# tub-rip/dvs_mcemvs

Hardware: AMD Instinct MI355X
Metric: Mevents/s into DSI (346x260x100) + DSI-fuse GB/s (higher is better)
Workload: dtype f32; 1 GPU; stereo (2-cam) synthetic DSEC-like rig, 10000000 events/cam per GPU, 346x260x100 DSI, harmonic camera fusion + arg-max; vote_algo=2, bands=10, band_rows=26, chunks=1, block_threads=1024, lds_bytes=74736, packed_lanes=7, parallelism=1 GPU, collective=none (1 rank), launched_by=single process, n_points=5000

## Files before the change

### dvs_mcemvs_amd/csrc/dsi_engine.cpp

```cpp
#include "../../include/dsi_engine.h"

#include <hip/hip_runtime.h>
#include <rccl/rccl.h>

#include <dlfcn.h>

#include <algorithm>
#include <atomic>
#include <chrono>
#include <cmath>
#include <cstdarg>
#include <cstdio>
#include <cstdlib>
#include <cstring>
#include <map>
#include <mutex>
#include <new>
#include <string>
#include <utility>
#include <vector>

#include "dsi_host.hpp"
#include "dsi_kernels.h"

// ... 295 lines not shown
    int algo = DSI_VOTE_AUTO;
    int want_band_rows = 0, want_chunks = 0, want_block = 0;
    int want_packed = -1;
    bool keep_z0 = false;
    dsi_vote_info_t info{};
    DevBuf<float> centers, H, Rt_tmp, conf, depth;
    DevBuf<unsigned long long> partials;
    DevBuf<float2> xy;
    DevBuf<dsi::EvRec> sxy;
    DevBuf<unsigned long long> seam;
    DevBuf<uint32_t> nvalid, cuts, gcuts;
    size_t cuts_inline_min_packets = 8192;
    bool info_cuts_inline = false;
    DevBuf<uint8_t> spk;
    DevBuf<uint16_t> rowstart;
    DevBuf<dsi::PlaneCoef> coef;
    DevBuf<uint8_t> idx, conf8, mask, idx_filtered;
    DevBuf<uint32_t> minmax;
    bool depth_valid = false;
    bool filtered_valid = false;
    PcBuffers pc;
    struct BatchTables {
        DevBuf<float> centers;
        DevBuf<dsi::EvRec> sxy;
        DevBuf<uint32_t> nvalid, cuts;
        DevBuf<uint16_t> rowstart;
        DevBuf<dsi::PlaneCoef> coef;
        void release()
        {
            centers.release();
// ... 331 lines not shown
    dsi_grid* g = m->grid;
    const dsi::Geom& geom = m->geom;
    dsi::BandPlan bp{};
    int algo = m->algo;
    const bool can_band = plan_bands(m, np, &bp);
    if (algo == DSI_VOTE_AUTO) algo = can_band ? DSI_VOTE_LDS_BANDS : DSI_VOTE_GLOBAL_ATOMIC;
    if (algo == DSI_VOTE_LDS_BANDS && !can_band)
        return fail(DSI_ERR_INVALID, "grid rows of %d floats do not fit the LDS band kernel", geom.nx);

    m->info = dsi_vote_info_t{};
    m->info.algo = algo;
    m->info.n_packets = np;
    m->depth_valid = false;

    if (algo == DSI_VOTE_GLOBAL_ATOMIC) {
        if (int rc = stage_a()) return rc;
        if (int rc = prep_end(m, ps)) return rc;
        if (!accumulate) HIP_TRY(hipMemsetAsync(g->data, 0, g->n * sizeof(float), ctx->stream));
        VoteTimer vt(m);
        HIP_TRY(dsi::launch_vote_global(ctx->stream, xy, centers, (int)np, m->planes_dev, geom, g->data));
        vt.stop();
        return vote_done(m);
    }

    if ((np + 1) * dsi::kPacket * sizeof(dsi::EvRec) > 0xffffffffull) {
        if (bp.packed == 1 || bp.packed == 7) bp.packed = 3;
        if (bp.packed == 8) return fail(DSI_ERR_INVALID, "lane mapping 8 (paired cells) addresses records with 32 bits: %zu packets are too many", np);
        if (bp.packed == 4) bp.packed = 2;
        if (bp.packed == 5) bp.packed = 6;
    }

    m->info.bands = bp.bands;
    m->info.band_rows = bp.band_rows;
    m->info.chunks = bp.chunks;
    m->info.block_threads = bp.block_threads;
    m->info.lds_bytes = bp.lds_bytes;
    m->info.packed = bp.packed;
    m->info.group_packets = bp.group_packets;
    if (np == 0) {
        if (int rc = prep_end(m, ps)) return rc;
        if (!accumulate) HIP_TRY(hipMemsetAsync(g->data, 0, g->n * sizeof(float), ctx->stream));
        return vote_done(m);
    }
    HIP_TRY(m->sxy.reserve(np * dsi::kPacket + 1));
    HIP_TRY(m->nvalid.reserve(np + (size_t)geom.nz + 9));
    HIP_TRY(m->rowstart.reserve(np * (size_t)(geom.ny + 2 * bp.row_pad + 3) + 2));
    HIP_TRY(m->coef.reserve(np * geom.nz + 1));
    bp.rs_stride = (int)((np + 63) / 64 * 64);
    const bool rs_fits = (size_t)(geom.ny + 2 * bp.row_pad + 3) * (size_t)bp.rs_stride * 2 < ((size_t)1 << 32);
    bp.cuts_inline = ((bp.packed == 5 || bp.packed == 6) && np >= (size_t)m->cuts_inline_min_packets && rs_fits) ? 1 : 0;
    if (bp.cuts_inline)
        HIP_TRY(m->cuts.reserve(((size_t)(geom.ny + 2 * bp.row_pad + 3) * (size_t)bp.rs_stride + 1) / 2));
    else
        HIP_TRY(m->cuts.reserve(np * geom.nz * bp.bands));
    m->info_cuts_inline = bp.cuts_inline != 0;
    HIP_TRY(m->seam.reserve((size_t)bp.chunks * geom.nz * bp.bands * 2 * geom.nx));
    const bool direct = (bp.chunks == 1 && !accumulate);
    bp.raw_out = direct ? 0 : 1;
    if (!direct) HIP_TRY(m->partials.reserve((size_t)bp.chunks * dsi::partial_stride(g->n)));

    if (bp.packed == 2 || bp.packed == 4) {
        if (int rc = stage_a()) return rc;
        const int S = bp.group_packets;
        const size_t ngroups = (np + S - 1) / S;
        HIP_TRY(m->spk.reserve(np * dsi::kPacket));
        HIP_TRY(m->gcuts.reserve(ngroups * geom.nz * bp.bands));
        HIP_TRY(m->rowstart.reserve(ngroups * (size_t)(geom.ny + 2 * bp.row_pad + 3)));
        HIP_TRY(dsi::launch_sort_groups(ps, xy, (int)np, S, geom.ny, geom.nz, bp.row_pad, m->sxy.p, m->spk.p,
                                        m->nvalid.p, m->rowstart.p));
        HIP_TRY(dsi::launch_plane_coef(ps, centers, m->planes_dev, m->rowstart.p, m->nvalid.p, (int)np,
                                       geom, bp, m->coef.p, m->cuts.p));
        HIP_TRY(dsi::launch_group_cuts(ps, m->cuts.p, m->rowstart.p, (int)np, S, geom, bp, m->gcuts.p));
        if (int rc = prep_end(m, ps)) return rc;
        VoteTimer vt(m);
        HIP_TRY(dsi::launch_vote_groups(ctx->stream, m->sxy.p, m->spk.p, m->coef.p, m->gcuts.p, m->nvalid.p + np, (int)np, S, geom,
                                        bp, direct ? (void*)g->data : (void*)m->partials.p, m->seam.p));
        vt.stop();
    } else {
    if (raw && !m->keep_z0) {
        HIP_TRY(dsi::launch_sort_packets_raw(ps, raw->Rt, raw->x, raw->y, raw->first, m->lut_dev, m->sensor_w, m->sensor_h, geom,
                                             m->centers.p, (int)np, bp.row_pad, m->sxy.p, m->nvalid.p,
                                             m->rowstart.p, m->unit_multiplicity));
    } else {
        if (int rc = stage_a()) return rc;
        HIP_TRY(dsi::launch_sort_packets(ps, xy, (int)np, geom.ny, geom.nz, bp.row_pad, m->sxy.p, m->nvalid.p,
                                         m->rowstart.p));
    }
    HIP_TRY(dsi::launch_plane_coef(ps, centers, m->planes_dev, m->rowstart.p, m->nvalid.p, (int)np,
                                   geom, bp, m->coef.p, m->cuts.p));
    if (int rc = prep_end(m, ps)) return rc;
    VoteTimer vt(m);
    HIP_TRY(dsi::launch_vote_bands(ctx->stream, m->sxy.p, m->coef.p, m->cuts.p, m->nvalid.p + np, (int)np, geom, bp,
                                   direct ? (void*)g->data : (void*)m->partials.p, m->seam.p));
    vt.stop();
    }
    const bool fold = !direct && dsi::reduce_can_fold_seams(geom, g->n);
    if (!fold)
        HIP_TRY(dsi::launch_seam_rows(ctx->stream, m->seam.p, bp.chunks, geom, bp, direct ? (void*)g->data : (void*)m->partials.p));
    if (!direct)
        HIP_TRY(dsi::launch_reduce_partials(ctx->stream, m->partials.p, bp.chunks, g->n, g->data, accumulate ? 1 : 0,
                                            fold ? m->seam.p : nullptr, &geom, &bp));
    return vote_done(m);
}

bool same_shape(const dsi_grid* a, const dsi_grid* b)
{
    return a->nx == b->nx && a->ny == b->ny && a->nz == b->nz;
// ... 845 lines not shown
    m->fused_trace.release();
    m->fused_keys.release();
    m->pair_work.release();
    m->fused_splits.release();
    m->fused_prefix.release();
    m->Rt_tmp.release();
    m->conf.release();
    m->depth.release();
    m->xy.release();
    m->sxy.release();
    m->seam.release();
    m->nvalid.release();
    m->gcuts.release();
    m->spk.release();
    m->rowstart.release();
    m->cuts.release();
    m->coef.release();
    m->idx.release();
    m->conf8.release();
    m->mask.release();
    m->idx_filtered.release();
    m->minmax.release();
    m->pc.release();
    for (auto& t : m->alg2_tables) t.release();
    for (auto& pr : m->timing_pairs) {
        (void)hipEventDestroy(pr.first);
        (void)hipEventDestroy(pr.second);
    }
    for (hipEvent_t e : m->timing_pool) (void)hipEventDestroy(e);
    --m->ctx->children;
// ... 50 lines not shown
    return DSI_OK;
}

int dsi_mapper_set_packed_lanes(dsi_mapper_t* m, int mode)
{
    REQUIRE(m, DSI_ERR_INVALID, "mapper is null");
    REQUIRE(mode >= -1 && mode <= 8, DSI_ERR_INVALID, "mode must be -1 (auto) or 0..8");
    m->want_packed = mode;
    return DSI_OK;
}

int dsi_mapper_paired_overflow(dsi_mapper_t* m, int* overflowed)
{
    REQUIRE(m && overflowed, DSI_ERR_INVALID, "null argument");
    *overflowed = 0;
    if (m->info.algo != DSI_VOTE_LDS_BANDS || m->info.packed != 8 || m->info.n_packets == 0) return DSI_OK;
    if (int rc = set_device(m->ctx)) return rc;
    uint32_t word = 0;
    HIP_TRY(hipStreamSynchronize(m->ctx->stream));
    HIP_TRY(hipMemcpy(&word, m->nvalid.p + m->info.n_packets + (size_t)m->geom.nz + 8, sizeof word, hipMemcpyDeviceToHost));
    *overflowed = word != 0u ? 1 : 0;
    return DSI_OK;
}

int dsi_mapper_set_inline_cuts(dsi_mapper_t* m, long long min_packets)
{
    REQUIRE(m, DSI_ERR_INVALID, "mapper is null");
    m->cuts_inline_min_packets = min_packets < 0 ? (size_t)8192 : (size_t)min_packets;
    return DSI_OK;
}

int dsi_mapper_fill_voxel_grid(dsi_mapper_t* m, const float* xy_z0, const float* centers, size_t n_packets)
{
    REQUIRE(m, DSI_ERR_INVALID, "mapper is null");
    REQUIRE(n_packets == 0 || (xy_z0 && centers), DSI_ERR_INVALID, "null input");
    REQUIRE(n_packets < ((size_t)1 << 21), DSI_ERR_INVALID, "too many packets in one call");
    dsi_context* ctx = m->ctx;
    if (int rc = set_device(ctx)) return rc;
    if (n_packets == 0) return DSI_OK;
    HIP_TRY(m->xy.reserve(n_packets * dsi::kPacket));
    HIP_TRY(m->centers.reserve(n_packets * 3));
    if (int rc = upload_async(ctx, m->xy.p, xy_z0, n_packets * dsi::kPacket * sizeof(float2))) return rc;
    if (int rc = upload_async(ctx, m->centers.p, centers, n_packets * 3 * sizeof(float))) return rc;
// ... 3101 lines not shown
```

### dvs_mcemvs_amd/csrc/dsi_kernels.h

```cpp
#pragma once

#include <hip/hip_runtime.h>
#include <stddef.h>
#include <stdint.h>

namespace dsi {

constexpr int kPacket = 1024;

struct PlaneCoef {
    float a, bx, by, d;
    float r;
    uint32_t flags;
    float d_a, by_a;
};
constexpr uint32_t kCoefSkip = 1u;
constexpr uint32_t kCoefSlow = 2u;
constexpr uint32_t kCoefInvertible = 4u;

struct EvRec {
    float x, y;
    uint32_t m;
};

// ... 12 lines not shown
    int chunks;
    int block_threads;
    int packed;
    int group_packets;
    int row_pad;
    int pass_lg;
    size_t lds_bytes;
    int scratch_offset;
    int persistent;
    int raw_out;
    int halo;
    int experiment;
    int interleave;
    int cuts_inline;
    int rs_stride;
};

inline int paired_row_words_host(int nx) { return 2 * ((nx >> 1) + 1); }

__host__ __device__ inline size_t partial_stride(size_t n_voxels) { return (n_voxels + 3) & ~(size_t)3; }

hipError_t launch_packet_geometry(hipStream_t s, const float* Rt, int np, const Geom& g,
                                  float* centers, float* H);
hipError_t launch_warp_z0(hipStream_t s, const uint16_t* ex, const uint16_t* ey,
                          const uint32_t* packet_first, int np, const float* H,
                          const float2* lut, int sensor_w, int sensor_h, float2* xy);
hipError_t launch_vote_global(hipStream_t s, const float2* xy, const float* centers, int np,
                              const float* planes, const Geom& g, float* dsi);
hipError_t launch_sort_packets_raw(hipStream_t s, const float* Rt, const uint16_t* ex, const uint16_t* ey,
                                   const uint32_t* packet_first, const float2* lut, int sensor_w, int sensor_h, const Geom& g,
                                   float* centers, int np, int pad, EvRec* sxy, uint32_t* nvalid,
                                   uint16_t* rowstart, int unit_multiplicity = 0);
hipError_t launch_sort_packets(hipStream_t s, const float2* xy, int np, int ny, int nz, int pad,
                               EvRec* sxy, uint32_t* nvalid, uint16_t* rowstart);
hipError_t launch_plane_coef(hipStream_t s, const float* centers, const float* planes,
                             const uint16_t* rowstart, uint32_t* nvalid, int np,
                             const Geom& g, const BandPlan& bp, PlaneCoef* coef, uint32_t* cuts);
hipError_t launch_vote_bands(hipStream_t s, const EvRec* sxy, const PlaneCoef* coef,
                             const uint32_t* cuts, const uint32_t* slow_any, int np, const Geom& g,
                             const BandPlan& bp, void* out, unsigned long long* seam);
hipError_t launch_seam_rows(hipStream_t s, const unsigned long long* seam, int chunks, const Geom& g,
                            const BandPlan& bp, void* out);
hipError_t launch_sort_groups(hipStream_t s, const float2* xy, int np, int S, int ny, int nz, int pad,
                              EvRec* sxy, uint8_t* spk, uint32_t* nvalid, uint16_t* rowstart);
hipError_t launch_group_cuts(hipStream_t s, const uint32_t* prow, const uint16_t* rowstart, int np,
                             int S, const Geom& g, const BandPlan& bp, uint32_t* gcuts);
hipError_t launch_vote_groups(hipStream_t s, const EvRec* sxy, const uint8_t* spk,
                              const PlaneCoef* coef, const uint32_t* gcuts, const uint32_t* slow_any,
                              int np, int S, const Geom& g, const BandPlan& bp, void* out, unsigned long long* seam);
hipError_t launch_reduce_partials(hipStream_t s, const unsigned long long* partials, int chunks, size_t n,
                                  float* dsi, int accumulate, const unsigned long long* seam = nullptr,
                                  const Geom* g = nullptr, const BandPlan* bp = nullptr);
inline bool reduce_can_fold_seams(const Geom& g, size_t n) { return (g.nx & 1) == 0 && n <= 0xffffffffull; }
struct FusedCamera {
    const EvRec* sxy;
// ... 232 lines not shown
```

### dvs_mcemvs_amd/csrc/dsi_kernels.hip

```cpp
#include "dsi_kernels.h"
#include "dsi_vote_asm.h"

#include <algorithm>
#include <atomic>
#include <cstdio>
#include <cstdlib>
#include <cmath>
#include <mutex>
#include <type_traits>
#include <vector>

#pragma clang fp contract(off)

namespace dsi {

namespace {

constexpr int kWave = 64;

__device__ __forceinline__ bool finitef(float v) { return __builtin_isfinite(v); }

__device__ __forceinline__ float dot3(float a0, float b0, float a1, float b1, float a2, float b2)
{
    const float x0 = a0 * b0, x1 = a1 * b1, x2 = a2 * b2;
// ... 198 lines not shown
    int np;
    EvRec* sxy;
    uint32_t* nvalid;
    uint16_t* rowstart;
    const float* planes;
    PlaneCoef* coef;
    uint32_t* cuts;
    uint32_t* pair_work;
};
struct PrepCameras {
    PrepCamera cam[kFusedMaxCameras];
    int n;
};

template <bool RAW>
__device__ __forceinline__ void sort_packets_body(const int k, const float2* __restrict__ xy, const RawEvents& raw,
                                                  int np, int ny,
                                                  int nz, int pad, EvRec* __restrict__ sxy,
                                                  uint32_t* __restrict__ nvalid,
                                                  uint16_t* __restrict__ rowstart, uint32_t* __restrict__ pair_work,
                                                  int n_pairs)
{
    extern __shared__ uint32_t hist[];
    __shared__ float s_H[9];
    __shared__ __attribute__((aligned(16))) unsigned long long hkey[kHashSlots];
    __shared__ uint32_t hcnt[RAW ? 1 : kHashSlots];
    __shared__ uint32_t wave_tot[4];
    __shared__ uint32_t big;
    const int nb = ny + 2 * pad + 2;
    if (k == 0) {
        for (int i = threadIdx.x; i < nz + 9; i += 256) nvalid[np + i] = 0;
        if (pair_work)
            for (int i = threadIdx.x; i < n_pairs; i += 256) pair_work[i] = 0;
        if (threadIdx.x == 0) {
            const EvRec none = {0.f, 0.f, 0u};
            sxy[(size_t)np * kPacket] = none;
        }
    }
    if (threadIdx.x == 0) big = 0;
    for (int i = threadIdx.x; i <= nb; i += 256) hist[i] = 0;
    for (int i = threadIdx.x; i < kHashSlots; i += 256) {
        hkey[i] = kHashEmpty;
        if (!RAW) hcnt[i] = 0;
    }
    if (RAW && threadIdx.x == 0) {
        float c3[3], h9[9];
        packet_geometry_of(raw.Rt + 12 * (size_t)k, raw.g, c3, h9);
#pragma unroll
        for (int i = 0; i < 3; ++i) raw.centers[3 * (size_t)k + i] = c3[i];
#pragma unroll
        for (int i = 0; i < 9; ++i) s_H[i] = h9[i];
    }
    float2 ev[4];
    uint32_t pixel4[4] = {0u, 0u, 0u, 0u};
    if (RAW) {
        const size_t first_ev = raw.packet_first ? (size_t)raw.packet_first[k] : (size_t)k * kPacket;
        unsigned px[4], py[4];
#pragma unroll
        for (int h = 0; h < 4; ++h) {
            const size_t e = first_ev + threadIdx.x + 256 * h;
            px[h] = raw.ex[e];
            py[h] = raw.ey[e];
        }
#pragma unroll
// ... 78 lines not shown
        if (lane >= off) incl += v;
    }
    if (lane == 63) wave_tot[threadIdx.x >> 6] = incl;
    __syncthreads();
    uint32_t base = incl - local;
    for (int w = 0; w < (int)(threadIdx.x >> 6); ++w) base += wave_tot[w];
    const uint32_t total = wave_tot[0] + wave_tot[1] + wave_tot[2] + wave_tot[3];
    __syncthreads();
    for (int i = b0; i < b1; ++i) {
        const uint32_t c = hist[i];
        hist[i] = base;
        base += c;
    }
    if (threadIdx.x == 0) hist[nb] = total;
    __syncthreads();
    uint16_t* rs = rowstart + (size_t)k * (nb + 1);
    for (int i = threadIdx.x; i <= nb; i += 256) rs[i] = (uint16_t)hist[i];
    static_assert(sizeof(unsigned long long) * kHashSlots >= sizeof(EvRec) * kPacket, "staging area");
    EvRec* stage = reinterpret_cast<EvRec*>(hkey);
#pragma unroll
    for (int h = 0; h < 4; ++h)
        if (bin[h] >= 0) {
            EvRec r;
            r.x = ev[h].x;
            r.y = ev[h].y;
            r.m = mult[h];
            stage[hist[bin[h]] + rank[h]] = r;
        }
    __syncthreads();
    {
        const int n16 = (int)((total * (uint32_t)sizeof(EvRec) + 15u) / 16u);
        const uint4* src = reinterpret_cast<const uint4*>(stage);
        uint4* dst = reinterpret_cast<uint4*>(sxy + (size_t)k * kPacket);
        for (int i = threadIdx.x; i < n16; i += 256) dst[i] = src[i];
    }
    if (threadIdx.x == 0) nvalid[k] = total | (big << 31);
}

template <bool RAW>
__global__ __launch_bounds__(256) __attribute__((amdgpu_waves_per_eu(8, 8))) void k_sort_packets(const float2* __restrict__ xy, RawEvents raw,
                                                      int np, int ny,
                                                      int nz, int pad, EvRec* __restrict__ sxy,
                                                      uint32_t* __restrict__ nvalid,
                                                      uint16_t* __restrict__ rowstart)
{
    sort_packets_body<RAW>((int)blockIdx.x, xy, raw, np, ny, nz, pad, sxy, nvalid, rowstart, nullptr, 0);
}

__global__ __launch_bounds__(256) __attribute__((amdgpu_waves_per_eu(8, 8))) void k_sort_packets_multi(PrepCameras cams, int ny, int nz, int pad,
                                                                                                       int n_pairs)
{
// ... 17 lines not shown
    ymax += m;
    const float fa = fminf(fmaxf(__builtin_floorf(ymin), (float)(-pad - 1)), (float)(ny + pad));
    const float fb = fminf(fmaxf(__builtin_floorf(ymax), (float)(-pad - 1)), (float)(ny + pad));
    *bin_lo = (int)fa + pad + 1;
    *bin_hi = (int)fb + pad + 2;
    return true;
}
__device__ __forceinline__ void band_y_interval(int j, const Geom& g, const BandPlan& bp, float* L, float* U)
{
    const int r0 = j * bp.band_rows;
    const int r1 = min(g.ny, r0 + bp.band_rows);
    *L = (float)(r0 - bp.halo) - 0.01f;
    *U = (float)min(r1, g.ny - 1) + 0.01f;
}

template <bool STAGED>
__device__ __forceinline__ void plane_coef_body(const unsigned bid, const float* __restrict__ centers,
                                                const float* __restrict__ planes,
                                                const uint16_t* __restrict__ rowstart,
                                                uint32_t* __restrict__ nvalid, int np,
                                                const Geom& g, const BandPlan& bp,
                                                PlaneCoef* __restrict__ coef,
                                                uint32_t* __restrict__ cuts, uint32_t* __restrict__ pair_work)
{
    extern __shared__ uint16_t s_rowstart[];
    const int tiles_p = (np + kCoefTilePackets - 1) / kCoefTilePackets;
    const unsigned tile = (bid >> 6) * 64u + (bid & 7u) * 8u + ((bid >> 3) & 7u);
    const int planes_per_block = (int)(blockDim.x >> 4);
    if (tile >= (unsigned)tiles_p * (unsigned)((g.nz + planes_per_block - 1) / planes_per_block)) return;
    const int k0 = (int)(tile % (unsigned)tiles_p) * kCoefTilePackets;
    const int k = k0 + (int)(threadIdx.x & 15);
    const int z = (int)(tile / (unsigned)tiles_p) * planes_per_block + (int)(threadIdx.x >> 4);
    const int pad = bp.row_pad;
    const int nb = g.ny + 2 * pad + 2;
    if (STAGED && !(bp.cuts_inline && !pair_work)) {
        const int count = min(kCoefTilePackets, np - k0) * (nb + 1);
        const uint32_t* src = reinterpret_cast<const uint32_t*>(rowstart + (size_t)k0 * (nb + 1));
        uint32_t* dst = reinterpret_cast<uint32_t*>(s_rowstart);
        for (int i = threadIdx.x; i < (count + 1) / 2; i += blockDim.x) dst[i] = src[i];
        __syncthreads();
    }
    const bool valid = k < np && z < g.nz;
    if (!valid && !pair_work) return;
    const int kq = valid ? k : 0, zq = valid ? z : 0;
    const size_t tid = (size_t)zq * np + kq;
    PlaneCoef c;
    plane_coefficients(centers[3 * kq], centers[3 * kq + 1], centers[3 * kq + 2], planes[zq], g, c.a,
                       c.bx, c.by, c.d);
    c.r = 1.f / c.d;
    const uint32_t nvraw = !valid ? 0u : (grouped(bp.packed) ? 1u : nvalid[kq]);
    const int nv = (int)(nvraw & 0x7fffffffu);
    const bool big_events = (nvraw >> 31) != 0;
    const bool dead = !(c.a == c.a) || !(c.bx == c.bx) || !(c.by == c.by) || !(c.d == c.d) ||
                      c.d == 0.f || !finitef(c.a) || !finitef(c.bx) || !finitef(c.by) || nv == 0;
    const float ad = fabsf(c.d);
    const bool slow = !dead && (!(ad >= 0x1p-40f && ad <= 0x1p40f)  ||
                                big_events || fabsf(c.a) > 0x1p40f || fabsf(c.bx) > 0x1p40f ||
                                fabsf(c.by) > 0x1p40f);
    const double a = (double)c.a, d = (double)c.d, by = (double)c.by;
    const bool invertible = !dead && !slow && fabs(a) > 1e-3 * fabs(d);
    const double inv_a = 1.0 / a;
    const float by_a = (float)(by * inv_a), d_a = (float)(d * inv_a);
    const float margin = 2e-5f * ((float)(g.ny + 1) * fabsf(d_a) + 2.f * fabsf(by_a));
    const bool inline_ok = invertible && fabsf(d_a) <= 1e4f && fabsf(by_a) <= 1e8f && margin <= 200.f;
    const uint32_t margin_q = inline_ok ? (uint32_t)__builtin_ceilf(margin * 256.f) + 1u : 0u;
    c.flags = (dead ? kCoefSkip : (slow ? kCoefSlow : 0u)) | (inline_ok ? kCoefInvertible : 0u) | (margin_q << 16);
    c.d_a = d_a;
    c.by_a = by_a;
    if (valid) coef[tid] = c;
    if (slow) atomicOr(&nvalid[np + zq], 1u);
    if (bp.cuts_inline && !pair_work) return;

    const uint16_t* rs = STAGED ? s_rowstart + (size_t)(threadIdx.x & 15) * (nb + 1)
                                : rowstart + (grouped(bp.packed) ? 0 : (size_t)kq * (nb + 1));
    for (int j = 0; j < bp.bands; ++j) {
        uint32_t lo = 0, hi = 0;
        if (!dead) {
            hi = (uint32_t)nv;
            if (invertible) {
                float L, U;
                band_y_interval(j, g, bp, &L, &U);
                int bin_lo, bin_hi;
                if (band_row_bins(d_a, by_a, L, U, g.ny, pad, &bin_lo, &bin_hi)) {
                    if (grouped(bp.packed)) {
                        lo = (uint32_t)bin_lo;
                        hi = (uint32_t)bin_hi;
                    } else {
                        lo = rs[bin_lo];
                        hi = rs[bin_hi];
                    }
                } else if (grouped(bp.packed)) {
                    lo = 0;
                    hi = (uint32_t)nb;
                }
            } else if (grouped(bp.packed)) {
                lo = 0;
                hi = (uint32_t)nb;
            }
            if (hi < lo) hi = lo;
        } else if (grouped(bp.packed)) {
            lo = 0xffffu;
            hi = 0;
        }
        if (valid && !bp.cuts_inline) cuts[((size_t)j * g.nz + zq) * np + kq] = lo | (hi << 16);
        if (pair_work) {
            int len = (int)hi - (int)lo;
            len += __builtin_amdgcn_update_dpp(0, len, 0x111, 0xf, 0xf, true);
            len += __builtin_amdgcn_update_dpp(0, len, 0x112, 0xf, 0xf, true);
            len += __builtin_amdgcn_update_dpp(0, len, 0x114, 0xf, 0xf, true);
            len += __builtin_amdgcn_update_dpp(0, len, 0x118, 0xf, 0xf, true);
            if ((threadIdx.x & 15) == 15 && len > 0 && z < g.nz) atomicAdd(&pair_work[j * g.nz + z], (uint32_t)len);
        }
    }
}

template <bool STAGED>
__global__ __launch_bounds__(1024) void k_plane_coef(const float* __restrict__ centers,
                                                    const float* __restrict__ planes,
                                                    const uint16_t* __restrict__ rowstart,
                                                    uint32_t* __restrict__ nvalid, int np,
                                                    Geom g, BandPlan bp,
// ... 8 lines not shown
};

template <bool STAGED>
__global__ __launch_bounds__(1024) void k_plane_coef_multi(PrepCameras cams, BandPlan bp, PrepBlocks blocks)
{
    unsigned bid = blockIdx.x;
    int c = 0;
#pragma unroll
    for (int k = 0; k < kFusedMaxCameras - 1; ++k)
        if (c == k && cams.n > k + 1 && bid >= blocks.n[k]) {
            bid -= blocks.n[k];
            c = k + 1;
        }
    const PrepCamera& pc = cams.cam[c];
    plane_coef_body<STAGED>(bid, pc.raw.centers, pc.planes, pc.rowstart, pc.nvalid, pc.np, pc.raw.g, bp, pc.coef, pc.cuts, pc.pair_work);
}

__global__ __launch_bounds__(256) void k_transpose_rowstart(const uint16_t* __restrict__ rs, int np, int nb1, int stride,
                                                            uint16_t* __restrict__ rsT)
{
    __shared__ uint16_t tile[64][66];
    const int p0 = (int)blockIdx.x * 64, b0 = (int)blockIdx.y * 64;
    {
        const int bin = b0 + (int)(threadIdx.x & 63);
        for (int i = (int)(threadIdx.x >> 6); i < 64; i += 4) {
            const int p = p0 + i;
            tile[i][threadIdx.x & 63] = (p < np && bin < nb1) ? rs[(size_t)p * nb1 + bin] : (uint16_t)0;
        }
    }
    __syncthreads();
// ... 1471 lines not shown
            s_pass = 2 * (BLOCK / kWave);
        }
        __syncthreads();
    }
    for (;;) {
    const int b = work_counters ? s_item : (int)blockIdx.x;
    if (b >= total) break;
    int q, z;
    if (!item_of(b, pairs, g.nz, q, z, bp.experiment == 200)) {
        if (!work_counters) break;
        __syncthreads();
        if (threadIdx.x == 0) s_item = (int)atomicAdd(&work_counters[cls], 1u) * 8 + cls;
        __syncthreads();
        continue;
    }
    if (work_counters && threadIdx.x == 0) s_next = (int)atomicAdd(&work_counters[cls], 1u) * 8 + cls;
    const int c = q / bp.bands, j = q % bp.bands;
    const int r0 = j * bp.band_rows;
    const int r1 = min(g.ny, r0 + bp.band_rows);
    const int cells = (r1 - r0 + 1) * row_words;
    if (!work_counters) {
        for (int i = threadIdx.x; i < cells; i += BLOCK) band[i] = 0;
        if (threadIdx.x == 0) s_pass = 2 * (BLOCK / kWave);
        __syncthreads();
    }

    const int p_begin = (int)(((long long)np * c) / bp.chunks);
    const int p_end = (int)(((long long)np * (c + 1)) / bp.chunks);
    if (bp.experiment != 1)
        stream_item<BLOCK, MAPPING>(sxy, coef, cuts, slow_any, np, g, bp, j, z, p_begin, p_end,
// ... 2335 lines not shown
        hipLaunchKernelGGL(k_transpose_rowstart, dim3((unsigned)(bp.rs_stride / 64), (unsigned)((nb1 + 63) / 64)), dim3(256), 0, s,
                           rowstart, np, nb1, bp.rs_stride, reinterpret_cast<uint16_t*>(cuts));
        return hipExtGetLastError();
    }
    if (!grouped(bp.packed) && table_bytes <= max_dynamic_lds()) {
        if (hipError_t e = allow_dynamic_lds(reinterpret_cast<const void*>(&k_plane_coef<true>), table_bytes)) return e;
        hipLaunchKernelGGL(k_plane_coef<true>, dim3((tiles_p * (unsigned)((g.nz + 63) / 64) + 63u) & ~63u), dim3(1024), table_bytes, s,
                           centers, planes, rowstart, nvalid, np, g, bp, coef, cuts);
    } else {
        hipLaunchKernelGGL(k_plane_coef<false>, dim3((tiles_p * (unsigned)((g.nz + 15) / 16) + 63u) & ~63u), dim3(256), 0, s, centers,
                           planes, rowstart, nvalid, np, g, bp, coef, cuts);
    }
    return hipExtGetLastError();
}

template <int BLOCK, int MAPPING>
static hipError_t launch_vote_bands_t(hipStream_t s, const EvRec* sxy, const PlaneCoef* coef,
                                      const uint32_t* cuts, const uint32_t* slow_any, int np,
                                      const Geom& g, const BandPlan& bp, void* out, unsigned long long* seam)
{
    constexpr bool PACKED = MAPPING != 0;
    constexpr bool VFILL = MAPPING == 5 || MAPPING == 6;
    const void* kern = VFILL ? reinterpret_cast<const void*>(&k_vote_bands_vfill<BLOCK, (VFILL ? MAPPING : 5)>)
                     : PACKED ? reinterpret_cast<const void*>(&k_vote_bands_packed<BLOCK, (PACKED && !VFILL ? MAPPING : 1)>)
                              : reinterpret_cast<const void*>(&k_vote_bands<BLOCK>);
    if (hipError_t e = allow_dynamic_lds(kern, bp.lds_bytes)) return e;
    unsigned blocks = (unsigned)item_count(bp.chunks * bp.bands, g.nz, bp.experiment == 200);
    uint32_t* counters = nullptr;
    if (PACKED && bp.persistent) {
        int dev = 0, cus = 256;
// ... 3420 lines not shown
```

### dvs_mcemvs_amd/engine.py

```python
import atexit
import ctypes as C
import os
import sys
import weakref

import numpy as np

PACKET_SIZE = 1024

FUSE_MIN, FUSE_HM, FUSE_GM, FUSE_AM, FUSE_RMS, FUSE_MAX = 1, 2, 3, 4, 5, 6
ACC_SUM, ACC_INV_SUM, ACC_LOG_SUM, ACC_SQ_SUM, ACC_MIN, ACC_MAX, ACC_GM_TREE = 0, 1, 2, 3, 4, 5, 6
REDUCE_SUM, REDUCE_MIN, REDUCE_MAX = 0, 1, 2
VOTE_AUTO, VOTE_GLOBAL_ATOMIC, VOTE_LDS_BANDS, VOTE_FUSED_ARGMAX = 0, 1, 2, 3
FOCUS_LOCAL_VAR, FOCUS_LOCAL_MS, FOCUS_GRAD_MAG, FOCUS_LAPLACIAN, FOCUS_DOG = 0, 1, 2, 3, 4
GRID_OP_SUBTRACT, GRID_OP_RATIO, GRID_OP_QUADRATIC_MEAN, GRID_OP_CUBIC_MEAN = 1, 2, 3, 4
LENS_PLUMB_BOB, LENS_FISHEYE = 0, 1

(OK, ERR_INVALID, ERR_TOO_FEW_EVENTS, ERR_HIP, ERR_SHAPE, ERR_BAD_OP, ERR_NO_DEVICE,
 ERR_CONTEXT, ERR_COMM) = range(9)
COMM_ID_BYTES = 128

_HERE = os.path.dirname(os.path.abspath(__file__))
_LIB = None

# ... 143 lines not shown
        "dsi_grid_slices_u8": (C.c_int, [vp, C.c_uint, C.c_int, u8p]),
        "dsi_grid_slices_u8_dev": (C.c_int, [vp, C.c_uint, C.c_int, vp]),
        "dsi_grid_laplacian": (C.c_int, [vp]),
        "dsi_grid_smooth_diffuse": (C.c_int, [vp, C.c_float, intp]),
        "dsi_grid_smooth_iir": (C.c_int, [vp, C.c_float, C.c_float, C.c_float, C.c_int]),
        "dsi_grid_mean_std": (C.c_int, [vp, f64p, f64p]),
        "dsi_grid_moran_index": (C.c_int, [vp, C.c_float, f64p]),
        "dsi_mapper_create": (C.c_int, [vp, C.POINTER(_MapperConfig), C.POINTER(vp)]),
        "dsi_mapper_destroy": (C.c_int, [vp]),
        "dsi_mapper_grid": (vp, [vp]),
        "dsi_mapper_geometry": (C.c_int, [vp, f32p, f32p, intp, intp, intp]),
        "dsi_mapper_set_vote_algo": (C.c_int, [vp, C.c_int]),
        "dsi_mapper_set_band_params": (C.c_int, [vp, C.c_int, C.c_int, C.c_int]),
        "dsi_mapper_set_packed_lanes": (C.c_int, [vp, C.c_int]),
        "dsi_mapper_set_inline_cuts": (C.c_int, [vp, C.c_longlong]),
        "dsi_mapper_paired_overflow": (C.c_int, [vp, C.POINTER(C.c_int)]),
        "dsi_mapper_fill_voxel_grid": (C.c_int, [vp, f32p, f32p, C.c_size_t]),
        "dsi_batch_create": (C.c_int, [vp, u16p, u16p, C.c_size_t, u32p, f32p, C.c_size_t,
                                       C.POINTER(vp)]),
        "dsi_batch_destroy": (C.c_int, [vp]),
        "dsi_batch_create_async": (C.c_int, [vp, u16p, u16p, C.c_size_t, u32p, f32p, C.c_size_t,
                                             C.POINTER(vp)]),
        "dsi_batch_uploaded": (C.c_int, [vp]),
        "dsi_host_alloc": (C.c_int, [C.c_size_t, C.POINTER(vp)]),
        "dsi_host_free": (C.c_int, [vp]),
        "dsi_mapper_fetch_depth_map_async": (C.c_int, [vp, f32p, f32p, u8p]),
        "dsi_mapper_fetch_depth_map_in_order": (C.c_int, [vp, f32p, f32p, u8p]),
        "dsi_mapper_fetch_wait": (C.c_int, [vp]),
        "dsi_batch_num_packets": (C.c_size_t, [vp]),
        "dsi_mapper_evaluate_batch": (C.c_int, [vp, vp]),
# ... 1133 lines not shown
    def set_band_params(self, band_rows=0, chunks=0, block_threads=0):
        _check(load_library().dsi_mapper_set_band_params(self._h, int(band_rows), int(chunks),
                                                         int(block_threads)))

    def set_packed_lanes(self, mode=-1):
        _check(load_library().dsi_mapper_set_packed_lanes(self._h, int(mode)))

    def paired_overflow(self):
        flag = C.c_int(0)
        _check(load_library().dsi_mapper_paired_overflow(self._h, C.byref(flag)))
        return bool(flag.value)

    def set_inline_cuts(self, min_packets=-1):
        _check(load_library().dsi_mapper_set_inline_cuts(self._h, int(min_packets)))

    def last_vote_info(self):
        info = _VoteInfo()
        _check(load_library().dsi_mapper_last_vote_info(self._h, C.byref(info)))
        return {k: getattr(info, k) for k, _ in _VoteInfo._fields_}

    def vote_statistics(self, batch):
        a, r = C.c_double(), C.c_double()
        _check(load_library().dsi_mapper_vote_statistics(self._h, batch._h, C.byref(a), C.byref(r)))
        return a.value, r.value

    def set_kernel_timing(self, enable=True):
        _check(load_library().dsi_mapper_set_kernel_timing(self._h, 1 if enable else 0))

    def vote_kernel_time(self):
        ms, n = C.c_float(), C.c_int()
# ... 324 lines not shown
```

### include/dsi_engine.h

```cpp
#ifndef DSI_ENGINE_H
#define DSI_ENGINE_H

#include <stddef.h>
#include <stdint.h>

#ifdef __cplusplus
extern "C" {
#endif

#if defined(__GNUC__)
#define DSI_API __attribute__((visibility("default")))
#else
#define DSI_API
#endif

#define DSI_ENGINE_ABI_VERSION 10
#define DSI_PACKET_SIZE 1024

typedef enum {
    DSI_OK = 0,
    DSI_ERR_INVALID = 1,
    DSI_ERR_TOO_FEW_EVENTS = 2,
    DSI_ERR_HIP = 3,
    DSI_ERR_SHAPE = 4,
// ... 137 lines not shown
    int plane_begin;
    int plane_count;
} dsi_mapper_config_t;

DSI_API int dsi_mapper_create(dsi_context_t *ctx, const dsi_mapper_config_t *cfg, dsi_mapper_t **out);
DSI_API int dsi_mapper_destroy(dsi_mapper_t *m);
DSI_API dsi_grid_t *dsi_mapper_grid(dsi_mapper_t *m);
DSI_API int dsi_mapper_geometry(const dsi_mapper_t *m, float *Kv, float *raw_depths, int *nx, int *ny, int *nz);
DSI_API int dsi_mapper_plane_begin(const dsi_mapper_t *m);
DSI_API int dsi_mapper_full_depths(const dsi_mapper_t *m, float *raw_depths, int *dim_z);
DSI_API int dsi_mapper_set_vote_algo(dsi_mapper_t *m, int algo);
DSI_API int dsi_mapper_set_band_params(dsi_mapper_t *m, int band_rows, int chunks, int block_threads);
DSI_API int dsi_mapper_set_packed_lanes(dsi_mapper_t *m, int mode);
DSI_API int dsi_mapper_paired_overflow(dsi_mapper_t *m, int *overflowed);
DSI_API int dsi_mapper_set_inline_cuts(dsi_mapper_t *m, long long min_packets);

DSI_API int dsi_mapper_fill_voxel_grid(dsi_mapper_t *m, const float *xy_z0, const float *centers, size_t n_packets);

DSI_API int dsi_batch_create(dsi_context_t *ctx, const uint16_t *x, const uint16_t *y, size_t n_events,
                     const uint32_t *packet_first, const float *Rt, size_t n_packets, dsi_batch_t **out);
DSI_API int dsi_host_alloc(size_t bytes, void **out);
DSI_API int dsi_host_free(void *p);
DSI_API int dsi_batch_create_async(dsi_context_t *ctx, const uint16_t *x, const uint16_t *y, size_t n_events,
                           const uint32_t *packet_first, const float *Rt, size_t n_packets, dsi_batch_t **out);
DSI_API int dsi_batch_uploaded(const dsi_batch_t *b);
DSI_API int dsi_batch_destroy(dsi_batch_t *b);
DSI_API size_t dsi_batch_num_packets(const dsi_batch_t *b);

DSI_API int dsi_mapper_evaluate_batch(dsi_mapper_t *m, const dsi_batch_t *batch);

// ... 246 lines not shown
```

Before: 7759 Mevents/s.

## Add one-launch packet preparation kernel and far-first plane ordering in band vote

Adds an optional fused kernel that sorts raw events per packet and computes plane coefficients and band cuts in the same launch. It uses double-buffered slow flags so the next call's flags are cleared inside the kernel. The aim is to drop the separate plane_coef launch and the rowstart round-trip through global memory. Separately, the band vote kernel now processes depth planes in reverse order by default, which changes the work scheduling order. The fused path is opt-in and adds API surface and complexity.

```diff
diff --git a/dvs_mcemvs_amd/csrc/dsi_engine.cpp b/dvs_mcemvs_amd/csrc/dsi_engine.cpp
--- a/dvs_mcemvs_amd/csrc/dsi_engine.cpp
+++ b/dvs_mcemvs_amd/csrc/dsi_engine.cpp
@@ -333,6 +333,11 @@
     bool info_cuts_inline = false;
     DevBuf<uint8_t> spk;
     DevBuf<uint16_t> rowstart;
+    int fused_prepare = -1;
+    DevBuf<uint32_t> prep_flags;
+    int prep_flags_next = -1;
+    size_t prep_flags_words = 0;
+    const uint32_t* slow_any = nullptr;
     DevBuf<dsi::PlaneCoef> coef;
     DevBuf<uint8_t> idx, conf8, mask, idx_filtered;
     DevBuf<uint32_t> minmax;
@@ -694,6 +699,8 @@
     m->depth_valid = false;
 
     if (algo == DSI_VOTE_GLOBAL_ATOMIC) {
+        if (m->fused_prepare == 1 && np)
+            return fail(DSI_ERR_INVALID, "the one-launch preparation belongs to the LDS band kernels, not to global atomics");
         if (int rc = stage_a()) return rc;
         if (int rc = prep_end(m, ps)) return rc;
         if (!accumulate) HIP_TRY(hipMemsetAsync(g->data, 0, g->n * sizeof(float), ctx->stream));
@@ -724,7 +731,6 @@
     }
     HIP_TRY(m->sxy.reserve(np * dsi::kPacket + 1));
     HIP_TRY(m->nvalid.reserve(np + (size_t)geom.nz + 9));
-    HIP_TRY(m->rowstart.reserve(np * (size_t)(geom.ny + 2 * bp.row_pad + 3) + 2));
     HIP_TRY(m->coef.reserve(np * geom.nz + 1));
     bp.rs_stride = (int)((np + 63) / 64 * 64);
     const bool rs_fits = (size_t)(geom.ny + 2 * bp.row_pad + 3) * (size_t)bp.rs_stride * 2 < ((size_t)1 << 32);
@@ -734,6 +740,15 @@
     else
         HIP_TRY(m->cuts.reserve(np * geom.nz * bp.bands));
     m->info_cuts_inline = bp.cuts_inline != 0;
+    bp.far_first = 1;
+    const bool can_fuse_prepare = raw && !m->keep_z0 && dsi::prepare_packets_applies(geom, bp);
+    if (m->fused_prepare == 1 && !can_fuse_prepare)
+        return fail(DSI_ERR_INVALID, "the one-launch preparation needs raw events and lane mapping 1, 3, 7 or 8 with a cut table "
+                                     "(this call: mapping %d%s)", bp.packed, raw ? "" : ", z0 locations");
+    const bool fuse_prepare = can_fuse_prepare && m->fused_prepare == 1;
+    if (!fuse_prepare)
+        HIP_TRY(m->rowstart.reserve(np * (size_t)(geom.ny + 2 * bp.row_pad + 3) + 2));
+    m->slow_any = m->nvalid.p + np;
     HIP_TRY(m->seam.reserve((size_t)bp.chunks * geom.nz * bp.bands * 2 * geom.nx));
     const bool direct = (bp.chunks == 1 && !accumulate);
     bp.raw_out = direct ? 0 : 1;
@@ -757,6 +772,24 @@
                                         bp, direct ? (void*)g->data : (void*)m->partials.p, m->seam.p));
         vt.stop();
     } else {
+    if (fuse_prepare) {
+        const size_t words = (size_t)geom.nz + 9;
+        if (m->prep_flags.cap < 2 * words || m->prep_flags_words != words) m->prep_flags_next = -1;
+        HIP_TRY(m->prep_flags.reserve(2 * words));
+        if (m->prep_flags_next < 0) {
+            HIP_TRY(hipMemsetAsync(m->prep_flags.p, 0, 2 * words * sizeof(uint32_t), ps));
+            m->prep_flags_words = words;
+            m->prep_flags_next = 0;
+        }
+        uint32_t* flags = m->prep_flags.p + (size_t)m->prep_flags_next * words;
+        uint32_t* next_flags = m->prep_flags.p + (size_t)(m->prep_flags_next ^ 1) * words;
+        m->prep_flags_next = -1;
+        HIP_TRY(dsi::launch_prepare_packets(ps, raw->Rt, raw->x, raw->y, raw->first, m->lut_dev, m->sensor_w, m->sensor_h, geom, bp,
+                                            m->centers.p, m->planes_dev, (int)np, m->sxy.p, m->nvalid.p, nullptr, flags, next_flags,
+                                            m->coef.p, m->cuts.p, nullptr, m->unit_multiplicity));
+        m->prep_flags_next = (int)((next_flags - m->prep_flags.p) / (ptrdiff_t)words);
+        m->slow_any = flags;
+    } else {
     if (raw && !m->keep_z0) {
         HIP_TRY(dsi::launch_sort_packets_raw(ps, raw->Rt, raw->x, raw->y, raw->first, m->lut_dev, m->sensor_w, m->sensor_h, geom,
                                              m->centers.p, (int)np, bp.row_pad, m->sxy.p, m->nvalid.p,
@@ -768,9 +801,10 @@
     }
     HIP_TRY(dsi::launch_plane_coef(ps, centers, m->planes_dev, m->rowstart.p, m->nvalid.p, (int)np,
                                    geom, bp, m->coef.p, m->cuts.p));
+    }
     if (int rc = prep_end(m, ps)) return rc;
     VoteTimer vt(m);
-    HIP_TRY(dsi::launch_vote_bands(ctx->stream, m->sxy.p, m->coef.p, m->cuts.p, m->nvalid.p + np, (int)np, geom, bp,
+    HIP_TRY(dsi::launch_vote_bands(ctx->stream, m->sxy.p, m->coef.p, m->cuts.p, m->slow_any, (int)np, geom, bp,
                                    direct ? (void*)g->data : (void*)m->partials.p, m->seam.p));
     vt.stop();
     }
@@ -1646,6 +1680,7 @@
     m->gcuts.release();
     m->spk.release();
     m->rowstart.release();
+    m->prep_flags.release();
     m->cuts.release();
     m->coef.release();
     m->idx.release();
@@ -1726,11 +1761,11 @@
 {
     REQUIRE(m && overflowed, DSI_ERR_INVALID, "null argument");
     *overflowed = 0;
-    if (m->info.algo != DSI_VOTE_LDS_BANDS || m->info.packed != 8 || m->info.n_packets == 0) return DSI_OK;
+    if (m->info.algo != DSI_VOTE_LDS_BANDS || m->info.packed != 8 || m->info.n_packets == 0 || !m->slow_any) return DSI_OK;
     if (int rc = set_device(m->ctx)) return rc;
     uint32_t word = 0;
     HIP_TRY(hipStreamSynchronize(m->ctx->stream));
-    HIP_TRY(hipMemcpy(&word, m->nvalid.p + m->info.n_packets + (size_t)m->geom.nz + 8, sizeof word, hipMemcpyDeviceToHost));
+    HIP_TRY(hipMemcpy(&word, m->slow_any + (size_t)m->geom.nz + 8, sizeof word, hipMemcpyDeviceToHost));
     *overflowed = word != 0u ? 1 : 0;
     return DSI_OK;
 }
@@ -1739,6 +1774,14 @@
 {
     REQUIRE(m, DSI_ERR_INVALID, "mapper is null");
     m->cuts_inline_min_packets = min_packets < 0 ? (size_t)8192 : (size_t)min_packets;
+    return DSI_OK;
+}
+
+int dsi_mapper_set_fused_prepare(dsi_mapper_t* m, int mode)
+{
+    REQUIRE(m, DSI_ERR_INVALID, "mapper is null");
+    REQUIRE(mode >= -1 && mode <= 1, DSI_ERR_INVALID, "mode must be -1 (auto), 0 (two launches) or 1 (one launch)");
+    m->fused_prepare = mode;
     return DSI_OK;
 }
 
diff --git a/dvs_mcemvs_amd/csrc/dsi_kernels.h b/dvs_mcemvs_amd/csrc/dsi_kernels.h
--- a/dvs_mcemvs_amd/csrc/dsi_kernels.h
+++ b/dvs_mcemvs_amd/csrc/dsi_kernels.h
@@ -50,6 +50,7 @@
     int interleave;
     int cuts_inline;
     int rs_stride;
+    int far_first;
 };
 
 inline int paired_row_words_host(int nx) { return 2 * ((nx >> 1) + 1); }
@@ -75,6 +76,12 @@
 hipError_t launch_vote_bands(hipStream_t s, const EvRec* sxy, const PlaneCoef* coef,
                              const uint32_t* cuts, const uint32_t* slow_any, int np, const Geom& g,
                              const BandPlan& bp, void* out, unsigned long long* seam);
+bool prepare_packets_applies(const Geom& g, const BandPlan& bp);
+hipError_t launch_prepare_packets(hipStream_t s, const float* Rt, const uint16_t* ex, const uint16_t* ey,
+                                  const uint32_t* packet_first, const float2* lut, int sensor_w, int sensor_h, const Geom& g,
+                                  const BandPlan& bp, float* centers, const float* planes, int np, EvRec* sxy, uint32_t* nvalid,
+                                  uint16_t* rowstart, uint32_t* flags, uint32_t* next_flags, PlaneCoef* coef, uint32_t* cuts,
+                                  uint32_t* pair_work = nullptr, int unit_multiplicity = 0);
 hipError_t launch_seam_rows(hipStream_t s, const unsigned long long* seam, int chunks, const Geom& g,
                             const BandPlan& bp, void* out);
 hipError_t launch_sort_groups(hipStream_t s, const float2* xy, int np, int S, int ny, int nz, int pad,
diff --git a/dvs_mcemvs_amd/csrc/dsi_kernels.hip b/dvs_mcemvs_amd/csrc/dsi_kernels.hip
--- a/dvs_mcemvs_amd/csrc/dsi_kernels.hip
+++ b/dvs_mcemvs_amd/csrc/dsi_kernels.hip
@@ -236,22 +236,24 @@
 };
 
 template <bool RAW>
-__device__ __forceinline__ void sort_packets_body(const int k, const float2* __restrict__ xy, const RawEvents& raw,
-                                                  int np, int ny,
-                                                  int nz, int pad, EvRec* __restrict__ sxy,
-                                                  uint32_t* __restrict__ nvalid,
-                                                  uint16_t* __restrict__ rowstart, uint32_t* __restrict__ pair_work,
-                                                  int n_pairs)
+__device__ __forceinline__ uint32_t sort_packets_body(const int k, const float2* __restrict__ xy, const RawEvents& raw,
+                                                      int np, int ny,
+                                                      int nz, int pad, EvRec* __restrict__ sxy,
+                                                      uint32_t* __restrict__ nvalid,
+                                                      uint16_t* __restrict__ rowstart, uint32_t* __restrict__ pair_work,
+                                                      int n_pairs, uint32_t* __restrict__ next_flags = nullptr,
+                                                      float* __restrict__ center_out = nullptr)
 {
     extern __shared__ uint32_t hist[];
-    __shared__ float s_H[9];
+    __shared__ float s_H[12];
     __shared__ __attribute__((aligned(16))) unsigned long long hkey[kHashSlots];
     __shared__ uint32_t hcnt[RAW ? 1 : kHashSlots];
     __shared__ uint32_t wave_tot[4];
     __shared__ uint32_t big;
     const int nb = ny + 2 * pad + 2;
     if (k == 0) {
-        for (int i = threadIdx.x; i < nz + 9; i += 256) nvalid[np + i] = 0;
+        uint32_t* flags = next_flags ? next_flags : nvalid + np;
+        for (int i = threadIdx.x; i < nz + 9; i += 256) flags[i] = 0;
         if (pair_work)
             for (int i = threadIdx.x; i < n_pairs; i += 256) pair_work[i] = 0;
         if (threadIdx.x == 0) {
@@ -269,7 +271,7 @@
         float c3[3], h9[9];
         packet_geometry_of(raw.Rt + 12 * (size_t)k, raw.g, c3, h9);
 #pragma unroll
-        for (int i = 0; i < 3; ++i) raw.centers[3 * (size_t)k + i] = c3[i];
+        for (int i = 0; i < 3; ++i) raw.centers[3 * (size_t)k + i] = s_H[9 + i] = c3[i];
 #pragma unroll
         for (int i = 0; i < 9; ++i) s_H[i] = h9[i];
     }
@@ -378,8 +380,10 @@
     }
     if (threadIdx.x == 0) hist[nb] = total;
     __syncthreads();
-    uint16_t* rs = rowstart + (size_t)k * (nb + 1);
-    for (int i = threadIdx.x; i <= nb; i += 256) rs[i] = (uint16_t)hist[i];
+    if (rowstart) {
+        uint16_t* rs = rowstart + (size_t)k * (nb + 1);
+        for (int i = threadIdx.x; i <= nb; i += 256) rs[i] = (uint16_t)hist[i];
+    }
     static_assert(sizeof(unsigned long long) * kHashSlots >= sizeof(EvRec) * kPacket, "staging area");
     EvRec* stage = reinterpret_cast<EvRec*>(hkey);
 #pragma unroll
@@ -398,7 +402,13 @@
         uint4* dst = reinterpret_cast<uint4*>(sxy + (size_t)k * kPacket);
         for (int i = threadIdx.x; i < n16; i += 256) dst[i] = src[i];
     }
-    if (threadIdx.x == 0) nvalid[k] = total | (big << 31);
+    if (RAW && center_out) {
+#pragma unroll
+        for (int i = 0; i < 3; ++i) center_out[i] = s_H[9 + i];
+    }
+    const uint32_t nvraw = total | (big << 31);
+    if (threadIdx.x == 0) nvalid[k] = nvraw;
+    return nvraw;
 }
 
 template <bool RAW>
@@ -446,41 +456,12 @@
     *U = (float)min(r1, g.ny - 1) + 0.01f;
 }
 
-template <bool STAGED>
-__device__ __forceinline__ void plane_coef_body(const unsigned bid, const float* __restrict__ centers,
-                                                const float* __restrict__ planes,
-                                                const uint16_t* __restrict__ rowstart,
-                                                uint32_t* __restrict__ nvalid, int np,
-                                                const Geom& g, const BandPlan& bp,
-                                                PlaneCoef* __restrict__ coef,
-                                                uint32_t* __restrict__ cuts, uint32_t* __restrict__ pair_work)
-{
-    extern __shared__ uint16_t s_rowstart[];
-    const int tiles_p = (np + kCoefTilePackets - 1) / kCoefTilePackets;
-    const unsigned tile = (bid >> 6) * 64u + (bid & 7u) * 8u + ((bid >> 3) & 7u);
-    const int planes_per_block = (int)(blockDim.x >> 4);
-    if (tile >= (unsigned)tiles_p * (unsigned)((g.nz + planes_per_block - 1) / planes_per_block)) return;
-    const int k0 = (int)(tile % (unsigned)tiles_p) * kCoefTilePackets;
-    const int k = k0 + (int)(threadIdx.x & 15);
-    const int z = (int)(tile / (unsigned)tiles_p) * planes_per_block + (int)(threadIdx.x >> 4);
-    const int pad = bp.row_pad;
-    const int nb = g.ny + 2 * pad + 2;
-    if (STAGED && !(bp.cuts_inline && !pair_work)) {
-        const int count = min(kCoefTilePackets, np - k0) * (nb + 1);
-        const uint32_t* src = reinterpret_cast<const uint32_t*>(rowstart + (size_t)k0 * (nb + 1));
-        uint32_t* dst = reinterpret_cast<uint32_t*>(s_rowstart);
-        for (int i = threadIdx.x; i < (count + 1) / 2; i += blockDim.x) dst[i] = src[i];
-        __syncthreads();
-    }
-    const bool valid = k < np && z < g.nz;
-    if (!valid && !pair_work) return;
-    const int kq = valid ? k : 0, zq = valid ? z : 0;
-    const size_t tid = (size_t)zq * np + kq;
+__device__ __forceinline__ PlaneCoef plane_coef_of(float cx_, float cy_, float cz_, float zi, const Geom& g, uint32_t nvraw,
+                                                   bool* dead_out, bool* slow_out, bool* invertible_out)
+{
     PlaneCoef c;
-    plane_coefficients(centers[3 * kq], centers[3 * kq + 1], centers[3 * kq + 2], planes[zq], g, c.a,
-                       c.bx, c.by, c.d);
+    plane_coefficients(cx_, cy_, cz_, zi, g, c.a, c.bx, c.by, c.d);
     c.r = 1.f / c.d;
-    const uint32_t nvraw = !valid ? 0u : (grouped(bp.packed) ? 1u : nvalid[kq]);
     const int nv = (int)(nvraw & 0x7fffffffu);
     const bool big_events = (nvraw >> 31) != 0;
     const bool dead = !(c.a == c.a) || !(c.bx == c.bx) || !(c.by == c.by) || !(c.d == c.d) ||
@@ -499,44 +480,95 @@
     c.flags = (dead ? kCoefSkip : (slow ? kCoefSlow : 0u)) | (inline_ok ? kCoefInvertible : 0u) | (margin_q << 16);
     c.d_a = d_a;
     c.by_a = by_a;
-    if (valid) coef[tid] = c;
-    if (slow) atomicOr(&nvalid[np + zq], 1u);
-    if (bp.cuts_inline && !pair_work) return;
-
-    const uint16_t* rs = STAGED ? s_rowstart + (size_t)(threadIdx.x & 15) * (nb + 1)
-                                : rowstart + (grouped(bp.packed) ? 0 : (size_t)kq * (nb + 1));
-    for (int j = 0; j < bp.bands; ++j) {
-        uint32_t lo = 0, hi = 0;
-        if (!dead) {
-            hi = (uint32_t)nv;
-            if (invertible) {
-                float L, U;
-                band_y_interval(j, g, bp, &L, &U);
-                int bin_lo, bin_hi;
-                if (band_row_bins(d_a, by_a, L, U, g.ny, pad, &bin_lo, &bin_hi)) {
-                    if (grouped(bp.packed)) {
-                        lo = (uint32_t)bin_lo;
-                        hi = (uint32_t)bin_hi;
-                    } else {
-                        lo = rs[bin_lo];
-                        hi = rs[bin_hi];
-                    }
-                } else if (grouped(bp.packed)) {
-                    lo = 0;
-                    hi = (uint32_t)nb;
+    *dead_out = dead;
+    *slow_out = slow;
+    *invertible_out = invertible;
+    return c;
+}
+
+template <typename RS>
+__device__ __forceinline__ uint32_t band_cut_of(int j, const Geom& g, const BandPlan& bp, int nv, bool dead, bool invertible,
+                                                float d_a, float by_a, const RS* __restrict__ rs)
+{
+    const int pad = bp.row_pad;
+    const int nb = g.ny + 2 * pad + 2;
+    uint32_t lo = 0, hi = 0;
+    if (!dead) {
+        hi = (uint32_t)nv;
+        if (invertible) {
+            float L, U;
+            band_y_interval(j, g, bp, &L, &U);
+            int bin_lo, bin_hi;
+            if (band_row_bins(d_a, by_a, L, U, g.ny, pad, &bin_lo, &bin_hi)) {
+                if (grouped(bp.packed)) {
+                    lo = (uint32_t)bin_lo;
+                    hi = (uint32_t)bin_hi;
+                } else {
+                    lo = rs[bin_lo];
+                    hi = rs[bin_hi];
                 }
             } else if (grouped(bp.packed)) {
                 lo = 0;
                 hi = (uint32_t)nb;
             }
-            if (hi < lo) hi = lo;
         } else if (grouped(bp.packed)) {
-            lo = 0xffffu;
-            hi = 0;
-        }
-        if (valid && !bp.cuts_inline) cuts[((size_t)j * g.nz + zq) * np + kq] = lo | (hi << 16);
+            lo = 0;
+            hi = (uint32_t)nb;
+        }
+        if (hi < lo) hi = lo;
+    } else if (grouped(bp.packed)) {
+        lo = 0xffffu;
+        hi = 0;
+    }
+    return lo | (hi << 16);
+}
+
+template <bool STAGED>
+__device__ __forceinline__ void plane_coef_body(const unsigned bid, const float* __restrict__ centers,
+                                                const float* __restrict__ planes,
+                                                const uint16_t* __restrict__ rowstart,
+                                                uint32_t* __restrict__ nvalid, int np,
+                                                const Geom& g, const BandPlan& bp,
+                                                PlaneCoef* __restrict__ coef,
+                                                uint32_t* __restrict__ cuts, uint32_t* __restrict__ pair_work)
+{
+    extern __shared__ uint16_t s_rowstart[];
+    const int tiles_p = (np + kCoefTilePackets - 1) / kCoefTilePackets;
+    const unsigned tile = (bid >> 6) * 64u + (bid & 7u) * 8u + ((bid >> 3) & 7u);
+    const int planes_per_block = (int)(blockDim.x >> 4);
+    if (tile >= (unsigned)tiles_p * (unsigned)((g.nz + planes_per_block - 1) / planes_per_block)) return;
+    const int k0 = (int)(tile % (unsigned)tiles_p) * kCoefTilePackets;
+    const int k = k0 + (int)(threadIdx.x & 15);
+    const int z = (int)(tile / (unsigned)tiles_p) * planes_per_block + (int)(threadIdx.x >> 4);
+    const int pad = bp.row_pad;
+    const int nb = g.ny + 2 * pad + 2;
+    if (STAGED && !(bp.cuts_inline && !pair_work)) {
+        const int count = min(kCoefTilePackets, np - k0) * (nb + 1);
+        const uint32_t* src = reinterpret_cast<const uint32_t*>(rowstart + (size_t)k0 * (nb + 1));
+        uint32_t* dst = reinterpret_cast<uint32_t*>(s_rowstart);
+        for (int i = threadIdx.x; i < (count + 1) / 2; i += blockDim.x) dst[i] = src[i];
+        __syncthreads();
+    }
+    const bool valid = k < np && z < g.nz;
+    if (!valid && !pair_work) return;
+    const int kq = valid ? k : 0, zq = valid ? z : 0;
+    const size_t tid = (size_t)zq * np + kq;
+    const uint32_t nvraw = !valid ? 0u : (grouped(bp.packed) ? 1u : nvalid[kq]);
+    const int nv = (int)(nvraw & 0x7fffffffu);
+    bool dead, slow, invertible;
+    const PlaneCoef c = plane_coef_of(centers[3 * kq], centers[3 * kq + 1], centers[3 * kq + 2], planes[zq], g, nvraw, &dead, &slow,
+                                      &invertible);
+    if (valid) coef[tid] = c;
+    if (slow) atomicOr(&nvalid[np + zq], 1u);
+    if (bp.cuts_inline && !pair_work) return;
+
+    const uint16_t* rs = STAGED ? s_rowstart + (size_t)(threadIdx.x & 15) * (nb + 1)
+                                : rowstart + (grouped(bp.packed) ? 0 : (size_t)kq * (nb + 1));
+    for (int j = 0; j < bp.bands; ++j) {
+        const uint32_t cut = band_cut_of(j, g, bp, nv, dead, invertible, c.d_a, c.by_a, rs);
+        if (valid && !bp.cuts_inline) cuts[((size_t)j * g.nz + zq) * np + kq] = cut;
         if (pair_work) {
-            int len = (int)hi - (int)lo;
+            int len = (int)(cut >> 16) - (int)(cut & 0xffffu);
             len += __builtin_amdgcn_update_dpp(0, len, 0x111, 0xf, 0xf, true);
             len += __builtin_amdgcn_update_dpp(0, len, 0x112, 0xf, 0xf, true);
             len += __builtin_amdgcn_update_dpp(0, len, 0x114, 0xf, 0xf, true);
@@ -575,6 +607,39 @@
         }
     const PrepCamera& pc = cams.cam[c];
     plane_coef_body<STAGED>(bid, pc.raw.centers, pc.planes, pc.rowstart, pc.nvalid, pc.np, pc.raw.g, bp, pc.coef, pc.cuts, pc.pair_work);
+}
+
+__global__ __launch_bounds__(256) __attribute__((amdgpu_waves_per_eu(8, 8))) void k_prepare_packets(
+    RawEvents raw, int np, BandPlan bp, int run, const float* __restrict__ planes, EvRec* __restrict__ sxy,
+    uint32_t* __restrict__ nvalid, uint16_t* __restrict__ rowstart, uint32_t* __restrict__ flags,
+    uint32_t* __restrict__ next_flags, PlaneCoef* __restrict__ coef, uint32_t* __restrict__ cuts,
+    uint32_t* __restrict__ pair_work)
+{
+    extern __shared__ uint32_t hist[];
+    const unsigned per_group = 8u * (unsigned)run, in_group = blockIdx.x % per_group;
+    const int k = (int)((blockIdx.x / per_group) * per_group + (in_group & 7u) * (unsigned)run + (in_group >> 3));
+    if (k >= np) return;
+    const Geom& g = raw.g;
+    float center[3];
+    const uint32_t nvraw = sort_packets_body<true>(k, nullptr, raw, np, g.ny, g.nz, bp.row_pad, sxy, nvalid, rowstart, nullptr, 0,
+                                                   next_flags, center);
+    const int nv = (int)(nvraw & 0x7fffffffu);
+    const int lg = g.nz >= 256 ? 8 : (g.nz <= 1 ? 0 : 32 - __builtin_clz((unsigned)g.nz - 1u));
+    const int group = (int)threadIdx.x >> lg, groups = 256 >> lg;
+    for (int z = (int)threadIdx.x & ((1 << lg) - 1); z < g.nz; z += 1 << lg) {
+        bool dead, slow, invertible;
+        const PlaneCoef c = plane_coef_of(center[0], center[1], center[2], planes[z], g, nvraw, &dead, &slow, &invertible);
+        if (group == 0) {
+            coef[(size_t)z * np + k] = c;
+            if (slow) atomicOr(&flags[z], 1u);
+        }
+        for (int j = group; j < bp.bands; j += groups) {
+            const uint32_t cut = band_cut_of(j, g, bp, nv, dead, invertible, c.d_a, c.by_a, hist);
+            cuts[((size_t)j * g.nz + z) * np + k] = cut;
+            const int len = (int)(cut >> 16) - (int)(cut & 0xffffu);
+            if (pair_work && len > 0) atomicAdd(&pair_work[j * g.nz + z], (uint32_t)len);
+        }
+    }
 }
 
 __global__ __launch_bounds__(256) void k_transpose_rowstart(const uint16_t* __restrict__ rs, int np, int nb1, int stride,
@@ -2076,6 +2141,7 @@
         __syncthreads();
         continue;
     }
+    if (bp.far_first) z = g.nz - 1 - z;
     if (work_counters && threadIdx.x == 0) s_next = (int)atomicAdd(&work_counters[cls], 1u) * 8 + cls;
     const int c = q / bp.bands, j = q % bp.bands;
     const int r0 = j * bp.band_rows;
@@ -4441,6 +4507,35 @@
     return hipExtGetLastError();
 }
 
+constexpr int kPrepareRun = 32;
+
+bool prepare_packets_applies(const Geom& g, const BandPlan& bp)
+{
+    const size_t table_bytes = ((size_t)kCoefTilePackets * (size_t)(g.ny + 2 * bp.row_pad + 3) * sizeof(uint16_t) + 7) & ~(size_t)7;
+    return (bp.packed == 1 || bp.packed == 3 || bp.packed == 7 || bp.packed == 8) && !bp.cuts_inline &&
+           table_bytes <= max_dynamic_lds();
+}
+
+hipError_t launch_prepare_packets(hipStream_t s, const float* Rt, const uint16_t* ex, const uint16_t* ey,
+                                  const uint32_t* packet_first, const float2* lut, int sensor_w, int sensor_h, const Geom& g,
+                                  const BandPlan& bp, float* centers, const float* planes, int np, EvRec* sxy, uint32_t* nvalid,
+                                  uint16_t* rowstart, uint32_t* flags, uint32_t* next_flags, PlaneCoef* coef, uint32_t* cuts,
+                                  uint32_t* pair_work, int unit_multiplicity)
+{
+    if (np <= 0) return hipSuccess;
+    if (!prepare_packets_applies(g, bp) || !flags || !next_flags || flags == next_flags) return hipErrorInvalidValue;
+    if (pair_work)
+        if (hipError_t e = hipMemsetAsync(pair_work, 0, (size_t)bp.bands * g.nz * sizeof(uint32_t), s)) return e;
+    const size_t lds = (size_t)(g.ny + 2 * bp.row_pad + 3) * sizeof(uint32_t);
+    RawEvents raw{Rt, ex, ey, packet_first, lut, sensor_w, sensor_h, g, centers, unit_multiplicity};
+    const int run = kPrepareRun;
+    const unsigned per_group = 8u * (unsigned)run;
+    const unsigned blocks = ((unsigned)np + per_group - 1) / per_group * per_group;
+    hipLaunchKernelGGL(k_prepare_packets, dim3(blocks), dim3(256), lds, s, raw, np, bp, run, planes, sxy, nvalid, rowstart,
+                       flags, next_flags, coef, cuts, pair_work);
+    return hipExtGetLastError();
+}
+
 template <int BLOCK, int MAPPING>
 static hipError_t launch_vote_bands_t(hipStream_t s, const EvRec* sxy, const PlaneCoef* coef,
                                       const uint32_t* cuts, const uint32_t* slow_any, int np,
diff --git a/dvs_mcemvs_amd/engine.py b/dvs_mcemvs_amd/engine.py
--- a/dvs_mcemvs_amd/engine.py
+++ b/dvs_mcemvs_amd/engine.py
@@ -181,6 +181,7 @@
         "dsi_mapper_set_band_params": (C.c_int, [vp, C.c_int, C.c_int, C.c_int]),
         "dsi_mapper_set_packed_lanes": (C.c_int, [vp, C.c_int]),
         "dsi_mapper_set_inline_cuts": (C.c_int, [vp, C.c_longlong]),
+        "dsi_mapper_set_fused_prepare": (C.c_int, [vp, C.c_int]),
         "dsi_mapper_paired_overflow": (C.c_int, [vp, C.POINTER(C.c_int)]),
         "dsi_mapper_fill_voxel_grid": (C.c_int, [vp, f32p, f32p, C.c_size_t]),
         "dsi_batch_create": (C.c_int, [vp, u16p, u16p, C.c_size_t, u32p, f32p, C.c_size_t,
@@ -1344,6 +1345,9 @@
     def set_inline_cuts(self, min_packets=-1):
         _check(load_library().dsi_mapper_set_inline_cuts(self._h, int(min_packets)))
 
+    def set_fused_prepare(self, mode=-1):
+        _check(load_library().dsi_mapper_set_fused_prepare(self._h, int(mode)))
+
     def last_vote_info(self):
         info = _VoteInfo()
         _check(load_library().dsi_mapper_last_vote_info(self._h, C.byref(info)))
diff --git a/include/dsi_engine.h b/include/dsi_engine.h
--- a/include/dsi_engine.h
+++ b/include/dsi_engine.h
@@ -175,6 +175,7 @@
 DSI_API int dsi_mapper_set_packed_lanes(dsi_mapper_t *m, int mode);
 DSI_API int dsi_mapper_paired_overflow(dsi_mapper_t *m, int *overflowed);
 DSI_API int dsi_mapper_set_inline_cuts(dsi_mapper_t *m, long long min_packets);
+DSI_API int dsi_mapper_set_fused_prepare(dsi_mapper_t *m, int mode);
 
 DSI_API int dsi_mapper_fill_voxel_grid(dsi_mapper_t *m, const float *xy_z0, const float *centers, size_t n_packets);
 
```

New measurement: 7778 Mevents/s (median of 6 runs). No clear change (+0.2%).
